# pnnl/ERT-Conditional-Diffusion-Model

Measured on AMD Instinct MI355X. Metric: denoising-steps/sec (64×64, batch 64) at 1/2/4/8 GPUs; conv HBM GB/s vs roofline, higher is better.
Workload: dtype f32

## Files before the change

### ert-conditional-diffusion-model_amd/csrc/unet_conv_wino4s.hip

```cpp
#include <cstdlib>
#include <type_traits>

#include "unet.h"

namespace ertd {
namespace unet {

namespace {

constexpr int NPW = 4;
constexpr int CCH = 8;
constexpr int NX = 36;
constexpr int VKS = 18 * 128;
constexpr int V_FL = 2 * VKS;
constexpr size_t WLDS = (size_t)2 * V_FL * sizeof(float);
constexpr int NRS = 3;
constexpr int GNC_JM = 4;
constexpr int GNC_KM = 6;
constexpr int GNC_TAB = 4096;
#ifndef WINO4S_PPRIO
#define WINO4S_PPRIO 2
#endif
#ifndef WINO4S_PD
#define WINO4S_PD 2
#endif
#ifndef WINO4S_MPRIO
#define WINO4S_MPRIO 1
#endif
#ifndef WINO4S_XCD
#define WINO4S_XCD 1
#endif
#ifndef WINO4S_XCDMAX
#define WINO4S_XCDMAX 2
#endif
#ifndef WINO4S_HALO
#define WINO4S_HALO 1
#endif
#ifndef WINO4S_ABL
#define WINO4S_ABL 0
#endif
using f32x4 = __attribute__((ext_vector_type(4))) float;
using f32x2 = __attribute__((ext_vector_type(2))) float;
using u32x4 = __attribute__((ext_vector_type(4))) unsigned;
using u32x2 = __attribute__((ext_vector_type(2))) unsigned;

__device__ __forceinline__ f32x2 fmac(f32x2 x, float c, f32x2 s) {
  return __builtin_elementwise_fma(x, f32x2{c, c}, s);
}
__device__ __forceinline__ void bt6(const float (&d)[6], float (&o)[6]) {
  const float c = d[4] - d[2], e = d[3] - d[1];
  const float u = d[4] - d[1], v = d[4] + d[1];
  o[0] = __builtin_fmaf(1.5f, e, __builtin_fmaf(-2.f, d[2], d[0] + d[4]));
  o[1] = __builtin_fmaf(2.5f, d[3], __builtin_fmaf(0.5f, d[2], u));
  o[2] = __builtin_fmaf(0.5f, d[3], __builtin_fmaf(-2.5f, d[2], v));
  o[3] = __builtin_fmaf(2.f, e, c);
  o[4] = __builtin_fmaf(-0.5f, e, c);
  o[5] = __builtin_fmaf(1.5f, c, __builtin_fmaf(-2.f, d[3], d[1] + d[5]));
}
__device__ __forceinline__ f32x2 pfma(f32x2 a, float c, f32x2 b) {
  return __builtin_elementwise_fma(a, f32x2{c, c}, b);
}
__device__ __forceinline__ void bt6p(const f32x2 (&d)[6], f32x2 (&o)[6]) {
  const f32x2 c = d[4] - d[2], e = d[3] - d[1];
  const f32x2 u = d[4] - d[1], v = d[4] + d[1];
  o[0] = pfma(e, 1.5f, pfma(d[2], -2.f, d[0] + d[4]));
  o[1] = pfma(d[3], 2.5f, pfma(d[2], 0.5f, u));
  o[2] = pfma(d[3], 0.5f, pfma(d[2], -2.5f, v));
  o[3] = pfma(e, 2.f, c);
  o[4] = pfma(e, -0.5f, c);
  o[5] = pfma(c, 1.5f, pfma(d[3], -2.f, d[1] + d[5]));
}
template <bool DEAD4>
__device__ __forceinline__ void bt6u(const float (&d)[6], float (&o)[6]) {
  const float c = d[4] - d[2], e = d[3] - d[1];
  o[0] = __builtin_fmaf(4.f, d[4], __builtin_fmaf(-5.f, d[2], d[0]));
  o[1] = __builtin_fmaf(-0.25f, d[1] + d[2], d[3] + d[4]);
  o[2] = __builtin_fmaf(0.5f, e, c);
  o[3] = __builtin_fmaf(-0.5f, e, c);
  o[4] = DEAD4 ? 0.f : __builtin_fmaf(0.25f, d[1] - d[2], d[4] - d[3]);
  o[5] = __builtin_fmaf(-1.25f, d[3], __builtin_fmaf(0.25f, d[1], d[5]));
}
template <bool DEAD4>
__device__ __forceinline__ void bt6pu(const f32x2 (&d)[6], f32x2 (&o)[6]) {
  const f32x2 c = d[4] - d[2], e = d[3] - d[1];
  o[0] = pfma(d[4], 4.f, pfma(d[2], -5.f, d[0]));
  o[1] = pfma(d[1] + d[2], -0.25f, d[3] + d[4]);
  o[2] = pfma(e, 0.5f, c);
  o[3] = pfma(e, -0.5f, c);
  o[4] = DEAD4 ? f32x2{0.f, 0.f} : pfma(d[1] - d[2], 0.25f, d[4] - d[3]);
  o[5] = pfma(d[3], -1.25f, pfma(d[1], 0.25f, d[5]));
}
__device__ __forceinline__ void at6u(const f32x2 (&m)[6], f32x2 (&y)[4]) {
  const f32x2 s = m[2] + m[3], d = m[2] - m[3];
  y[0] = (m[0] + m[1]) + s;
  y[1] = fmac(d, 0.5f, m[1]);
  y[2] = fmac(s, 0.25f, m[1]);
  y[3] = fmac(d, 0.125f, m[1] + m[5]);
}
template <int N, bool SHL>
__device__ __forceinline__ f32x2 row_shift0(f32x2 v) {
  constexpr int ctrl = (SHL ? 0x100 : 0x110) + N;
  return f32x2{__int_as_float(__builtin_amdgcn_update_dpp(0, __float_as_int(v.x), ctrl, 0xf, 0xf, true)),
               __int_as_float(__builtin_amdgcn_update_dpp(0, __float_as_int(v.y), ctrl, 0xf, 0xf, true))};
}
template <int N, bool SHL>
__device__ __forceinline__ f32x2 row_shift_keep(f32x2 old, f32x2 v) {
  constexpr int ctrl = (SHL ? 0x100 : 0x110) + N;
  return f32x2{__int_as_float(__builtin_amdgcn_update_dpp(__float_as_int(old.x), __float_as_int(v.x), ctrl, 0xf, 0xf, false)),
               __int_as_float(__builtin_amdgcn_update_dpp(__float_as_int(old.y), __float_as_int(v.y), ctrl, 0xf, 0xf, false))};
}
__device__ __forceinline__ void at6(const f32x2 (&m)[6], f32x2 (&y)[4]) {
  const f32x2 s = m[1] + m[2], d = m[1] - m[2];
  y[0] = (m[0] + s) + (m[3] + m[4]);
  y[1] = fmac(m[3], 0.5f, fmac(m[4], -2.f, d));
  y[2] = fmac(m[3], 0.25f, fmac(m[4], 4.f, s));
  y[3] = fmac(m[3], 0.125f, fmac(m[4], -8.f, d + m[5]));
}

#ifdef WINO4S_STAMP
constexpr int S4_SPW = 64;
__device__ unsigned g_w4s_stamps[256 * 12 * S4_SPW];
#define W4S_STAMP(slot)                                                                            \
  do {                                                                                             \
    if (blockIdx.x < 256 && lane == 0)                                                             \
      g_w4s_stamps[(blockIdx.x * 12 + wave) * S4_SPW + (slot)] = (unsigned)__builtin_amdgcn_s_memtime(); \
  } while (0)
#define W4S_STAMP_ENTRY()                                                                          \
  do {                                                                                             \
    if (blockIdx.x < 256 && lane == 0) {                                                           \
      g_w4s_stamps[(blockIdx.x * 12 + wave) * S4_SPW] = (unsigned)__builtin_amdgcn_s_memrealtime(); \
      g_w4s_stamps[(blockIdx.x * 12 + wave) * S4_SPW + 1] = (unsigned)__builtin_amdgcn_s_memtime(); \
    }                                                                                              \
  } while (0)
#else
#define W4S_STAMP(slot) \
  do {                  \
  } while (0)
#define W4S_STAMP_ENTRY() \
  do {                    \
  } while (0)
#endif

struct Item {
  int cog, blk, half;
};
__device__ __forceinline__ Item item_of(int it, int ncog, int ksp) {
  Item r;
  r.half = it % ksp;
  const int pr = it / ksp;
  r.cog = pr % ncog;
  r.blk = pr / ncog;
  return r;
}

struct ItemWalk {
  int bid, G, ncog, ksp;
  __device__ __forceinline__ Item at(int il) const { return item_of(bid + il * G, ncog, ksp); }
};

constexpr int up25_pair(int xh, int l) { return xh && l >= 3 ? l + 3 : l; }

template <int WO, int ACT, bool UP, int XS, bool GNC>
__global__ __launch_bounds__(64 * (4 * XS + NPW)) void conv_wino4s_kernel(ConvArgs a, int nitems, int ksp) {
  static_assert(!GNC || (XS == 2 && !UP && ACT != ACT_NONE), "GNC: the xi-split GN+act kernel");
  extern __shared__ __attribute__((aligned(16))) float smem[];
  float* vbuf = smem;

  constexpr int TPR = WO / 4;
  constexpr int HW = WO * WO;
  constexpr int TS = TPR * TPR;
  constexpr int WS = UP ? WO / 2 : WO;
  constexpr int HWS = WS * WS;
  constexpr bool UP25 = UP && XS == 2;
  static_assert(TS % 16 == 0 && TPR <= 16, "a 16-tile block is whole tile rows of one sample");
  const int tid = threadIdx.x;
  const int lane = tid & 63;
  const int wave = __builtin_amdgcn_readfirstlane(tid >> 6);
  W4S_STAMP_ENTRY();
  const int Cin = a.Cin, Ca = a.Ca;
  const int nchunk = Cin / CCH / ksp;
  const int ncog = a.Cout / 64;
  const int G = gridDim.x;
  const int bid = (WINO4S_XCD && G % 8 == 0 && ncog <= WINO4S_XCDMAX)
                      ? (int)(blockIdx.x % 8) * (G / 8) + (int)(blockIdx.x / 8) : (int)blockIdx.x;
  const ItemWalk wk{bid, G, ncog, ksp};
  const int nloc = bid < nitems ? (nitems - bid + G - 1) / G : 0;
  float2* const gtab = reinterpret_cast<float2*>(smem + 2 * V_FL + 4 * 2 * 8 * 256);
  const int gtot = nloc * nchunk;

  if (wave >= 4 * XS) {
    __builtin_amdgcn_s_setprio(WINO4S_PPRIO);
    const int q = wave - 4 * XS;
    const int chb = lane >> 5, h = (lane >> 4) & 1, t = lane & 15;
    const int cl = 2 * q + chb;
    const int vwoff = ((((cl >> 2) * 18 + 9 * h) * 4 + (cl & 3)) * 16 + t) * 2;
    const int nbaddr = (lane + 15 - 30 * h) * 4;
    const unsigned choff = (unsigned)(chb * HWS * 4);
    constexpr bool HALO = WINO4S_HALO && !UP && TPR <= 8;
    constexpr int NWR = HALO ? (TPR == 8 ? 5 : 4) : 6;
    float2 raw[NRS][NWR];
    float2 gnv[NRS];
    int gch[NRS];
    f32x4 pad[NRS];
    int cur_g = 0, cur_k = 0, cur_b = 0, cur_il = 0, cur_k0 = 0;
    unsigned roff[NWR];
    f32x4 cur_pad;
    auto set_item = [&](int il) {
      const Item itm = wk.at(il);
      cur_k0 = itm.half * nchunk;
      const int flat0 = itm.blk * 16;
      cur_b = flat0 / TS;
      const int tg = flat0 % TS + t;
      const int ty = tg / TPR, tx = tg - ty * TPR;
      if constexpr (UP) {
#pragma unroll
        for (int r = 0; r < 4; ++r) {
          const int sy = 2 * ty - 1 + r;
          roff[r] = (unsigned)(((sy >= 0 && sy < WS ? sy : 2 * ty) * WS + 2 * tx + h) * 4) + choff;
        }
      } else if constexpr (HALO) {
#pragma unroll
        for (int r = 0; r < 4; ++r) roff[r] = (unsigned)(((4 * ty + r) * WO + 4 * tx + 2 * h) * 4) + choff;
        if constexpr (TPR == 8) {
          const int iy = t < 8 ? 4 * ty - 1 : 4 * ty + 4;
          roff[4] = (unsigned)(((iy >= 0 && iy < WO ? iy : 4 * ty) * WO + 4 * tx + 2 * h) * 4) + choff;
        }
      } else {
#pragma unroll
        for (int r = 0; r < 6; ++r) {
          const int iy = 4 * ty - 1 + r;
          roff[r] = (unsigned)(((iy >= 0 && iy < WO ? iy : 4 * ty) * WO + 4 * tx + 2 * h) * 4) + choff;
        }
      }
      cur_pad = f32x4{ty > 0 ? 1.f : 0.f, ty < TPR - 1 ? 1.f : 0.f,
                      (h ? tx < TPR - 1 : tx > 0) ? 1.f : 0.f, 0.f};
    };
    const int glast = gtot - 1;
    auto load_next = [&](const int set) {
      const int cg = (cur_k0 + cur_k) * CCH + 2 * q;
      pad[set] = cur_pad;
      if constexpr (GNC) gch[set] = cur_il * Cin + cg + chb;
      else if constexpr (ACT != ACT_NONE) gnv[set] = a.gn[(size_t)cur_b * Cin + cg + chb];
      const bool inA = cg < Ca;
      const float* p = inA ? a.srcA + ((size_t)cur_b * Ca + cg) * HWS
                           : a.srcB + ((size_t)cur_b * a.Cb + (cg - Ca)) * HWS;
      const __amdgpu_buffer_rsrc_t rs =
          __builtin_amdgcn_make_buffer_rsrc(const_cast<float*>(p), (short)0, 2 * HWS * 4, 0x00020000);
      if constexpr (UP) {
        float v[4];
#pragma unroll
        for (int r = 0; r < 4; ++r) v[r] = __uint_as_float(__builtin_amdgcn_raw_buffer_load_b32(rs, (int)roff[r], 0, 0));
#pragma unroll
        for (int r = 0; r < 6; ++r) {
          const float u = v[(r + 1) >> 1];
          raw[set][r] = make_float2(u, u);
        }
      } else {
#pragma unroll
        for (int r = 0; r < NWR; ++r) {
          const auto v = __builtin_amdgcn_raw_buffer_load_b64(rs, (int)roff[r], 0, 0);
          raw[set][r] = make_float2(__uint_as_float(v[0]), __uint_as_float(v[1]));
        }
      }
      if (cur_g < glast) {
        ++cur_g;
        if (++cur_k == nchunk) {
          cur_k = 0;
          set_item(++cur_il);
        }
      }
    };
    f32x2 act2[2][6];
    float actn[2][6];
    auto act_stage = [&](const int set, const int ab) {
      if constexpr (GNC) gnv[set] = gtab[gch[set]];
      auto activate = [&](const float2 rw) {
        f32x2 v = f32x2{rw.x, rw.y};
        if constexpr (ACT != ACT_NONE) {
          v = __builtin_elementwise_fma(v, f32x2{gnv[set].x, gnv[set].x}, f32x2{gnv[set].y, gnv[set].y});
          if constexpr (ACT == ACT_GN_SILU) {
            f32x2 e = v * f32x2{-1.44269504088896340736f, -1.44269504088896340736f};
            e = f32x2{__builtin_amdgcn_exp2f(e.x), __builtin_amdgcn_exp2f(e.y)} + f32x2{1.0f, 1.0f};
            v = v * f32x2{__builtin_amdgcn_rcpf(e.x), __builtin_amdgcn_rcpf(e.y)};
          }
        }
        return v;
      };
      f32x2 m[6];
      if constexpr (HALO) {
#pragma unroll
        for (int r = 0; r < 4; ++r) m[1 + r] = activate(raw[set][r]);
        if constexpr (TPR == 8) {
          const f32x2 x = activate(raw[set][4]);
          m[0] = row_shift_keep<TPR, false>(x, m[4]);
          m[5] = row_shift_keep<TPR, true>(x, m[1]);
        } else {
          m[0] = row_shift0<TPR, false>(m[4]);
          m[5] = row_shift0<TPR, true>(m[1]);
        }
      } else {
#pragma unroll
        for (int r = 0; r < 6; ++r) m[r] = activate(raw[set][r]);
      }
      m[0] = m[0] * f32x2{pad[set].x, pad[set].x};
      m[5] = m[5] * f32x2{pad[set].y, pad[set].y};
      if constexpr (UP) bt6pu<UP25>(m, act2[ab]);
      else bt6p(m, act2[ab]);
#pragma unroll
      for (int i = 0; i < 6; ++i) {
        if constexpr (UP25) {
          if (i == 4) {
            actn[ab][i] = 0.f;
            continue;
          }
        }
        const float give = h ? act2[ab][i].y : act2[ab][i].x;
        const float nb = __int_as_float(__builtin_amdgcn_ds_bpermute(nbaddr, __float_as_int(give)));
        actn[ab][i] = nb * pad[set].z;
      }
    };
    auto tr_stage = [&](const int ab, float* vb) {
      float w[6][3];
#pragma unroll
      for (int i = 0; i < 6; ++i) {
        w[i][0] = act2[ab][i].x;
        w[i][1] = act2[ab][i].y;
        w[i][2] = actn[ab][i];
      }
      float row[3][6];
#pragma unroll
      for (int aa = 0; aa < 3; ++aa)
#pragma unroll
        for (int c = 0; c < 3; ++c) {
          const auto sw = __builtin_amdgcn_permlane16_swap(__float_as_uint(w[aa][c]),
                                                           __float_as_uint(w[3 + aa][c]), false, false);
          const int jl = c == 0 ? 1 : (c == 1 ? 2 : 0);
          row[aa][jl] = __uint_as_float(sw[0]);
          row[aa][3 + c] = __uint_as_float(sw[1]);
        }
      float* o = vb + vwoff;
#pragma unroll
      for (int aa = 0; aa < 3; ++aa) {
        float vv[6];
        if constexpr (UP) bt6u<UP25>(row[aa], vv);
        else bt6(row[aa], vv);
        if constexpr (UP25) {
          if (aa == 1 && h) continue;
        }
#pragma unroll
        for (int jp = 0; jp < 6; jp += 2)
          *reinterpret_cast<f32x2*>(o + (aa * 3 + jp / 2) * 128) = f32x2{vv[jp], vv[jp + 1]};
      }
    };
    auto slot = [&](auto sa, auto ab, int g) {
      constexpr int SA = decltype(sa)::value, AB = decltype(ab)::value;
      if constexpr (!(WINO4S_ABL & 1)) {
        tr_stage(AB ^ 1, vbuf + ((g + 1) & 1) * V_FL);
        act_stage(SA, AB);
      }
      load_next(SA);
      if constexpr (!(WINO4S_ABL & 16)) __syncthreads();
    };
    using I0 = std::integral_constant<int, 0>;
    using I1 = std::integral_constant<int, 1>;
    using I2 = std::integral_constant<int, 2>;
    if (gtot > 0) {
      set_item(0);
      load_next(0);
      load_next(1);
      load_next(2);
    }
    if constexpr (GNC) {
      W4S_STAMP(25);
      __syncthreads();
      W4S_STAMP(26);
    }
    if (gtot > 0) {
      act_stage(0, 0);
      tr_stage(0, vbuf);
      load_next(0);
      act_stage(1, 1);
      load_next(1);
    }
    W4S_STAMP(3);
    __syncthreads();
    W4S_STAMP(2);
    int g = 0;
    for (; g + 5 < gtot; g += 6) {
      slot(I2{}, I0{}, g);
      slot(I0{}, I1{}, g + 1);
      slot(I1{}, I0{}, g + 2);
      slot(I2{}, I1{}, g + 3);
      slot(I0{}, I0{}, g + 4);
      slot(I1{}, I1{}, g + 5);
    }
    if (g < gtot) slot(I2{}, I0{}, g);
    if (g + 1 < gtot) slot(I0{}, I1{}, g + 1);
    if (g + 2 < gtot) slot(I1{}, I0{}, g + 2);
    if (g + 3 < gtot) slot(I2{}, I1{}, g + 3);
    if (g + 4 < gtot) slot(I0{}, I0{}, g + 4);
    W4S_STAMP(27);
    return;
  }

  if constexpr (XS == 1) {
  const int cb = wave;
  f32x4 acc[NX];
  const int nks = Cin / 4;
  const __amdgpu_buffer_rsrc_t ru = __builtin_amdgcn_make_buffer_rsrc(
      const_cast<float*>(a.wpk_wino4), (short)0, (int)((size_t)NX * a.Cout * Cin * 4), 0x00020000);
  int u_il = 0, u_ks = 0;
  int u_base = 0;
  auto u_item = [&](int il) {
    const Item itm = wk.at(il);
    u_base = itm.cog * nks * 36864;
  };
  auto u_advance = [&]() {
    if (++u_ks == nks) {
      if (u_il + 1 < nloc) {
        u_ks = 0;
        u_item(++u_il);
      } else {
        u_ks = nks - 1;
      }
    }
  };
  if (nloc > 0) u_item(0);
  f32x2 ub[2][18];
  const int uvoff = lane * 8 + cb * 512;
  auto u_load = [&](f32x2 (&u)[18], const int p) {
    if constexpr ((WINO4S_ABL & 32) != 0) {
      u[p] = u[p] + f32x2{1.f, 1.f};
      return;
    }
    const auto v = __builtin_amdgcn_raw_buffer_load_b64(
        ru, uvoff, (WINO4S_ABL & 2) ? p * 2048 : u_base + u_ks * 36864 + p * 2048, 0);
    u[p] = f32x2{__uint_as_float(v[0]), __uint_as_float(v[1])};
  };
  if (nloc > 0) {
#pragma unroll
    for (int p = 0; p < 18; ++p) u_load(ub[0], p);
    u_advance();
  }
  __syncthreads();
#ifndef WINO4S_XK
#define WINO4S_XK 1
#endif
  auto kstep = [&](const f32x2 (&u)[18], f32x2 (&nx)[18], const float* vs) {
    constexpr int PD = WINO4S_PD;
    f32x2 rb[PD + 1];
#pragma unroll
    for (int p = 0; p < PD; ++p) rb[p] = *reinterpret_cast<const f32x2*>(vs + p * 128);
#pragma unroll
    for (int p = 0; p < 18; ++p) {
      if (p + PD < 18) rb[(p + PD) % (PD + 1)] = *reinterpret_cast<const f32x2*>(vs + (p + PD) * 128);
      const int r = p % (PD + 1);
      if constexpr (WINO4S_ABL & 4) {
        acc[2 * p][0] = __builtin_fmaf(u[p].x, rb[r].x, acc[2 * p][0]);
        acc[2 * p + 1][0] = __builtin_fmaf(u[p].y, rb[r].y, acc[2 * p + 1][0]);
      } else {
        acc[2 * p] = __builtin_amdgcn_mfma_f32_16x16x4f32(u[p].x, rb[r].x, acc[2 * p], 0, 0, 0);
        acc[2 * p + 1] = __builtin_amdgcn_mfma_f32_16x16x4f32(u[p].y, rb[r].y, acc[2 * p + 1], 0, 0, 0);
      }
      u_load(nx, p);
      if (p + PD < 18) __builtin_amdgcn_sched_group_barrier(0x100, 1, 0);
      __builtin_amdgcn_sched_group_barrier(0x008, 2, 0);
      __builtin_amdgcn_sched_group_barrier(0x020, 1, 0);
    }
    u_advance();
  };
  auto chunk2 = [&](const float* vs) {
    constexpr int PD = WINO4S_PD;
    f32x2 rb[PD + 1];
#pragma unroll
    for (int q = 0; q < PD; ++q) rb[q] = *reinterpret_cast<const f32x2*>(vs + q * 128);
#pragma unroll
    for (int q = 0; q < 36; ++q) {
      const int st = q / 18, p = q % 18;
      const int qn = q + PD;
      if (qn < 36) rb[qn % (PD + 1)] = *reinterpret_cast<const f32x2*>(vs + (qn / 18) * VKS + (qn % 18) * 128);
      const int r = q % (PD + 1);
      const f32x2 u = st == 0 ? ub[0][p] : ub[1][p];
      acc[2 * p] = __builtin_amdgcn_mfma_f32_16x16x4f32(u.x, rb[r].x, acc[2 * p], 0, 0, 0);
      acc[2 * p + 1] = __builtin_amdgcn_mfma_f32_16x16x4f32(u.y, rb[r].y, acc[2 * p + 1], 0, 0, 0);
      if (st == 0) u_load(ub[1], p);
      else u_load(ub[0], p);
      if (qn < 36) __builtin_amdgcn_sched_group_barrier(0x100, 1, 0);
      __builtin_amdgcn_sched_group_barrier(0x008, 2, 0);
      __builtin_amdgcn_sched_group_barrier(0x020, 1, 0);
      if (p == 17) u_advance();
    }
  };
  for (int il = 0; il < nloc; ++il) {
#pragma unroll
    for (int x = 0; x < NX; ++x) acc[x] = f32x4{};
    for (int k = 0; k < nchunk; ++k) {
      const int g = il * nchunk + k;
      int ln;
      asm volatile("v_mbcnt_lo_u32_b32 %0, -1, 0\n\tv_mbcnt_hi_u32_b32 %0, -1, %0" : "=v"(ln));
      const float* vb = vbuf + (g & 1) * V_FL + ln * 2;
      if constexpr (WINO4S_XK && !(WINO4S_ABL & 4)) {
        chunk2(vb);
      } else {
        kstep(ub[0], ub[1], vb);
        kstep(ub[1], ub[0], vb + VKS);
      }
#pragma unroll
      for (int x = 0; x < NX; ++x) asm volatile("" : "+v"(acc[x]));
      if constexpr (!(WINO4S_ABL & 16)) __syncthreads();
    }

    if constexpr ((WINO4S_ABL & 8) != 0) {
      if (il == nloc - 1) {
        float sacc = 0.f;
        for (int x = 0; x < NX; ++x) sacc += acc[x][0] + acc[x][3];
        a.out[(size_t)bid * 64 + lane] = sacc;
      }
      continue;
    }
    const Item itm = wk.at(il);
    const int flatw = itm.blk * 16;
    const int smpl = flatw / TS;
    const bool has_eb = a.ebias != nullptr, has_res = a.res != nullptr, has_bias = a.bias != nullptr;
    const unsigned smp = (unsigned)(a.Cout * HW * 4);
    const __amdgpu_buffer_rsrc_t ro = __builtin_amdgcn_make_buffer_rsrc(
        a.out + (size_t)smpl * a.Cout * HW, (short)0, smp, 0x00020000);
    const __amdgpu_buffer_rsrc_t rr = __builtin_amdgcn_make_buffer_rsrc(
        has_res ? const_cast<float*>(a.res) + (size_t)smpl * a.Cout * HW : nullptr, (short)0, smp,
        0x00020000);
    f32x4 y[4][4];
#pragma unroll
    for (int pp = 0; pp < 2; ++pp) {
      f32x2 P[6][4];
#pragma unroll
      for (int i = 0; i < 6; ++i) {
        f32x2 m[6];
#pragma unroll
        for (int j = 0; j < 6; ++j) m[j] = f32x2{acc[6 * i + j][2 * pp], acc[6 * i + j][2 * pp + 1]};
        if constexpr (UP) at6u(m, P[i]);
        else at6(m, P[i]);
      }
#pragma unroll
      for (int x = 0; x < 4; ++x) {
        f32x2 col[6], yc[4];
#pragma unroll
        for (int i = 0; i < 6; ++i) col[i] = P[i][x];
        if constexpr (UP) at6u(col, yc);
        else at6(col, yc);
#pragma unroll
        for (int r = 0; r < 4; ++r) {
          y[2 * pp][r][x] = yc[r].x;
          y[2 * pp + 1][r][x] = yc[r].y;
        }
      }
    }
    int ln;
    asm volatile("v_mbcnt_lo_u32_b32 %0, -1, 0\n\tv_mbcnt_hi_u32_b32 %0, -1, %0" : "=v"(ln));
    const int co0 = itm.cog * 64 + cb * 16 + 4 * (ln >> 4);
    const int tg = flatw % TS + (ln & 15);
    const int ty = tg / TPR, tx = tg - ty * TPR;
    const int vo = (co0 * HW + 4 * ty * WO + 4 * tx) * 4;
#pragma unroll
    for (int i = 0; i < 4; ++i) {
      const float bi = has_bias ? a.bias[co0 + i] : 0.f;
      const float ei = has_eb ? a.ebias[(size_t)smpl * a.eb_stride + co0 + i] : 0.f;
#pragma unroll
      for (int r = 0; r < 4; ++r) {
        y[i][r] = y[i][r] + bi;
        if (has_eb) y[i][r] = y[i][r] + ei;
      }
    }
    __builtin_amdgcn_sched_barrier(0);
    if (has_res) {
      f32x4 rv[4][4];
#pragma unroll
      for (int i = 0; i < 4; ++i)
#pragma unroll
        for (int r = 0; r < 4; ++r)
          rv[i][r] = __builtin_bit_cast(f32x4, __builtin_amdgcn_raw_buffer_load_b128(rr, vo, i * HW * 4 + r * WO * 4, 0));
#pragma unroll
      for (int i = 0; i < 4; ++i)
#pragma unroll
        for (int r = 0; r < 4; ++r) y[i][r] = y[i][r] + rv[i][r];
    }
    if (a.gnp) {
      float2 pr[4];
#pragma unroll
      for (int i = 0; i < 4; ++i) {
        float sm = 0.f;
#pragma unroll
        for (int r = 0; r < 4; ++r) sm += (y[i][r][0] + y[i][r][1]) + (y[i][r][2] + y[i][r][3]);
        sm = row16_sum(sm);
        const float mu = sm * (1.0f / 256.0f);
        float qq = 0.f;
#pragma unroll
        for (int r = 0; r < 4; ++r)
#pragma unroll
          for (int x = 0; x < 4; ++x) {
            const float d = y[i][r][x] - mu;
            qq = __builtin_fmaf(d, d, qq);
          }
        pr[i] = make_float2(sm, row16_sum(qq));
      }
      if ((ln & 15) == 0) {
        const int np = TS / 16, part = (flatw % TS) / 16;
#pragma unroll
        for (int i = 0; i < 4; ++i) {
          float2* d = a.gnp + ((size_t)smpl * a.Cout + co0 + i) * np + part;
          *d = pr[i];
        }
      }
    }
#pragma unroll
    for (int i = 0; i < 4; ++i)
#pragma unroll
      for (int r = 0; r < 4; ++r)
        __builtin_amdgcn_raw_buffer_store_b128(__builtin_bit_cast(u32x4, y[i][r]), ro, vo,
                                               i * HW * 4 + r * WO * 4, 0);
  }
  } else {
  constexpr int NP = 9;
  const int cb = wave & 3, xh = wave >> 2;
#if WINO4S_MPRIO
  if (xh) __builtin_amdgcn_s_setprio(WINO4S_MPRIO);
#endif
  float* xbuf = smem + 2 * V_FL;
  f32x4 acc[2 * NP];
  const int nks = Cin / 4;
  const __amdgpu_buffer_rsrc_t ru = __builtin_amdgcn_make_buffer_rsrc(
      const_cast<float*>(a.wpk_wino4), (short)0, (int)((size_t)NX * a.Cout * Cin * 4), 0x00020000);
  int u_il = 0, u_ks = 0, u_end = 0, u_base = 0;
  auto u_item = [&](int il) {
    const Item itm = wk.at(il);
    u_base = itm.cog * nks * 36864;
    u_ks = itm.half * nchunk * 2;
    u_end = u_ks + nchunk * 2;
  };
  auto u_advance = [&]() {
    if (++u_ks == u_end) {
      if (u_il + 1 < nloc) {
        u_item(++u_il);
      } else {
        u_ks = u_end - 1;
      }
    }
  };
  if (nloc > 0) u_item(0);
  f32x2 ub[2][NP];
  const int uvoff = lane * 8 + cb * 512;
  const int psoff = xh * NP * 2048;
  auto u_load = [&](f32x2 (&u)[NP], const int p) {
    const auto v = __builtin_amdgcn_raw_buffer_load_b64(ru, uvoff, u_base + u_ks * 36864 + psoff + p * 2048, 0);
    u[p] = f32x2{__uint_as_float(v[0]), __uint_as_float(v[1])};
  };
  if (nloc > 0) {
#pragma unroll
    for (int p = 0; p < NP; ++p) {
      if constexpr (UP25) {
        if (xh && p / 3 == 1) continue;
      }
      u_load(ub[0], p);
    }
    u_advance();
  }
  if constexpr (GNC) {
    constexpr int JM = GNC_JM;
    const int ng4 = (a.gnc.groups + 3) / 4;
    int smp[JM], jg[JM], row[JM];
    bool jl[JM];
#pragma unroll
    for (int j = 0; j < JM; ++j) {
      const int job = wave + 4 * XS * j, il = job / ng4;
      jl[j] = il < nloc;
      row[j] = jl[j] ? il : 0;
      jg[j] = job - il * ng4;
      smp[j] = jl[j] ? wk.at(il).blk * 16 / TS : 0;
    }
    gn_group_finalize_regs<JM, GNC_KM>(a.gnc, smp, jg, row, jl, lane, gtab);
    W4S_STAMP(25);
    __syncthreads();
    W4S_STAMP(26);
  }
  __syncthreads();
  W4S_STAMP(2);
  auto chunk2 = [&](const float* vs) {
    constexpr int PD = WINO4S_PD;
    f32x2 rb[PD + 1];
#pragma unroll
    for (int q = 0; q < PD; ++q) rb[q] = *reinterpret_cast<const f32x2*>(vs + (xh * NP + q) * 128);
#pragma unroll
    for (int q = 0; q < 2 * NP; ++q) {
      const int st = q / NP, p = q % NP;
      const int qn = q + PD;
      if (qn < 2 * NP)
        rb[qn % (PD + 1)] = *reinterpret_cast<const f32x2*>(vs + (qn / NP) * VKS + (xh * NP + qn % NP) * 128);
      const int r = q % (PD + 1);
      const f32x2 u = st == 0 ? ub[0][p] : ub[1][p];
      acc[2 * p] = __builtin_amdgcn_mfma_f32_16x16x4f32(u.x, rb[r].x, acc[2 * p], 0, 0, 0);
      acc[2 * p + 1] = __builtin_amdgcn_mfma_f32_16x16x4f32(u.y, rb[r].y, acc[2 * p + 1], 0, 0, 0);
      if (st == 0) u_load(ub[1], p);
      else u_load(ub[0], p);
      if (qn < 2 * NP) __builtin_amdgcn_sched_group_barrier(0x100, 1, 0);
      __builtin_amdgcn_sched_group_barrier(0x008, 2, 0);
      __builtin_amdgcn_sched_group_barrier(0x020, 1, 0);
      if (p == NP - 1) u_advance();
    }
  };
  auto chunk2u = [&](auto xhc, const float* vs) {
    constexpr int XH = decltype(xhc)::value;
    constexpr int NL = XH ? NP - 3 : NP;
    constexpr int PD = WINO4S_PD;
    f32x2 rb[PD + 1];
#pragma unroll
    for (int q = 0; q < PD; ++q) rb[q] = *reinterpret_cast<const f32x2*>(vs + (XH * NP + up25_pair(XH, q)) * 128);
#pragma unroll
    for (int q = 0; q < 2 * NL; ++q) {
      const int st = q / NL, p = up25_pair(XH, q % NL);
      const int qn = q + PD;
      if (qn < 2 * NL)
        rb[qn % (PD + 1)] =
            *reinterpret_cast<const f32x2*>(vs + (qn / NL) * VKS + (XH * NP + up25_pair(XH, qn % NL)) * 128);
      const int r = q % (PD + 1);
      const f32x2 u = st == 0 ? ub[0][p] : ub[1][p];
      const bool both = p % 3 != 2;
      if (both) acc[2 * p] = __builtin_amdgcn_mfma_f32_16x16x4f32(u.x, rb[r].x, acc[2 * p], 0, 0, 0);
      acc[2 * p + 1] = __builtin_amdgcn_mfma_f32_16x16x4f32(u.y, rb[r].y, acc[2 * p + 1], 0, 0, 0);
      if (st == 0) u_load(ub[1], p);
      else u_load(ub[0], p);
      if (qn < 2 * NL) __builtin_amdgcn_sched_group_barrier(0x100, 1, 0);
      if (both) __builtin_amdgcn_sched_group_barrier(0x008, 2, 0);
      else __builtin_amdgcn_sched_group_barrier(0x008, 1, 0);
      __builtin_amdgcn_sched_group_barrier(0x020, 1, 0);
      if (q % NL == NL - 1) u_advance();
    }
  };
  for (int il = 0; il < nloc; ++il) {
#pragma unroll
    for (int x = 0; x < 2 * NP; ++x) acc[x] = f32x4{};
    f32x2 own[4][4];
    auto tail_u = [&](auto xhc) {
      constexpr int XH = decltype(xhc)::value;
#pragma unroll
      for (int pp = 0; pp < 2; ++pp) {
        if (pp) __builtin_amdgcn_sched_barrier(0);
        f32x2 P[3][4], Y[4][4];
#pragma unroll
        for (int i = 0; i < 3; ++i) {
          if (XH && i == 1) continue;
          f32x2 m[6];
#pragma unroll
          for (int j = 0; j < 6; ++j)
            if (j != 4) m[j] = f32x2{acc[6 * i + j][2 * pp], acc[6 * i + j][2 * pp + 1]};
          m[4] = f32x2{0.f, 0.f};
          at6u(m, P[i]);
        }
#pragma unroll
        for (int x = 0; x < 4; ++x) {
          if constexpr (XH == 0) {
            Y[0][x] = P[0][x] + (P[1][x] + P[2][x]);
            Y[1][x] = fmac(P[2][x], 0.5f, P[1][x]);
            Y[2][x] = fmac(P[2][x], 0.25f, P[1][x]);
            Y[3][x] = fmac(P[2][x], 0.125f, P[1][x]);
          } else {
            Y[0][x] = P[0][x];
            Y[1][x] = P[0][x] * f32x2{-0.5f, -0.5f};
            Y[2][x] = P[0][x] * f32x2{0.25f, 0.25f};
            Y[3][x] = fmac(P[0][x], -0.125f, P[2][x]);
          }
        }
        if (pp == XH) {
#pragma unroll
          for (int r = 0; r < 4; ++r)
#pragma unroll
            for (int x = 0; x < 4; ++x) own[r][x] = Y[r][x];
        } else {
          float* xw = xbuf + ((cb * 2 + (XH ^ 1)) * 8) * 256 + lane * 4;
#pragma unroll
          for (int r = 0; r < 4; ++r)
#pragma unroll
            for (int x = 0; x < 4; x += 2)
              *reinterpret_cast<f32x4*>(xw + (r * 2 + x / 2) * 256) =
                  f32x4{Y[r][x].x, Y[r][x].y, Y[r][x + 1].x, Y[r][x + 1].y};
        }
      }
    };
    if (il < 8) W4S_STAMP(3 + 3 * il);
    auto kloop_u = [&](auto xhc) {
      for (int k = 0; k < nchunk; ++k) {
        const int g = il * nchunk + k;
        int ln;
        asm volatile("v_mbcnt_lo_u32_b32 %0, -1, 0\n\tv_mbcnt_hi_u32_b32 %0, -1, %0" : "=v"(ln));
        chunk2u(xhc, vbuf + (g & 1) * V_FL + ln * 2);
#pragma unroll
        for (int x = 0; x < 2 * NP; ++x)
          if (x % 6 != 4) asm volatile("" : "+v"(acc[x]));
        if (k == nchunk - 1) tail_u(xhc);
        __syncthreads();
#ifdef WINO4S_STAMP
        if (g < 32) W4S_STAMP(28 + g);
#endif
      }
    };
    if constexpr (UP25) {
      if (xh == 0) kloop_u(std::integral_constant<int, 0>{});
      else kloop_u(std::integral_constant<int, 1>{});
    } else {
    for (int k = 0; k < nchunk; ++k) {
      const int g = il * nchunk + k;
      int ln;
      asm volatile("v_mbcnt_lo_u32_b32 %0, -1, 0\n\tv_mbcnt_hi_u32_b32 %0, -1, %0" : "=v"(ln));
      chunk2(vbuf + (g & 1) * V_FL + ln * 2);
#pragma unroll
      for (int x = 0; x < 2 * NP; ++x) asm volatile("" : "+v"(acc[x]));
      if (k == nchunk - 1) {
#pragma unroll
        for (int pp = 0; pp < 2; ++pp) {
          f32x2 P[3][4];
#pragma unroll
          for (int i = 0; i < 3; ++i) {
            f32x2 m[6];
#pragma unroll
            for (int j = 0; j < 6; ++j) m[j] = f32x2{acc[6 * i + j][2 * pp], acc[6 * i + j][2 * pp + 1]};
            at6(m, P[i]);
          }
          f32x2 Y[4][4];
#pragma unroll
          for (int x = 0; x < 4; ++x) {
            if (xh == 0) {
              const f32x2 s12 = P[1][x] + P[2][x], d12 = P[1][x] - P[2][x];
              Y[0][x] = P[0][x] + s12;
              Y[1][x] = d12;
              Y[2][x] = s12;
              Y[3][x] = d12;
            } else {
              Y[0][x] = P[0][x] + P[1][x];
              Y[1][x] = fmac(P[0][x], 0.5f, P[1][x] * f32x2{-2.f, -2.f});
              Y[2][x] = fmac(P[0][x], 0.25f, P[1][x] * f32x2{4.f, 4.f});
              Y[3][x] = fmac(P[0][x], 0.125f, fmac(P[1][x], -8.f, P[2][x]));
            }
          }
          if (pp == xh) {
#pragma unroll
            for (int r = 0; r < 4; ++r)
#pragma unroll
              for (int x = 0; x < 4; ++x) own[r][x] = Y[r][x];
          } else {
            float* xw = xbuf + ((cb * 2 + (xh ^ 1)) * 8) * 256 + lane * 4;
#pragma unroll
            for (int r = 0; r < 4; ++r)
#pragma unroll
              for (int x = 0; x < 4; x += 2)
                *reinterpret_cast<f32x4*>(xw + (r * 2 + x / 2) * 256) =
                    f32x4{Y[r][x].x, Y[r][x].y, Y[r][x + 1].x, Y[r][x + 1].y};
          }
        }
      }
      __syncthreads();
#ifdef WINO4S_STAMP
      if (g < 32) W4S_STAMP(28 + g);
#endif
    }
    }
    if (il < 8) W4S_STAMP(4 + 3 * il);
    int ln;
    asm volatile("v_mbcnt_lo_u32_b32 %0, -1, 0\n\tv_mbcnt_hi_u32_b32 %0, -1, %0" : "=v"(ln));
    f32x4 y[2][4];
    {
      const float* xr = xbuf + ((cb * 2 + xh) * 8) * 256 + ln * 4;
#pragma unroll
      for (int r = 0; r < 4; ++r)
#pragma unroll
        for (int x = 0; x < 4; x += 2) {
          const f32x4 o = *reinterpret_cast<const f32x4*>(xr + (r * 2 + x / 2) * 256);
          const f32x2 q0 = own[r][x] + f32x2{o[0], o[1]}, q1 = own[r][x + 1] + f32x2{o[2], o[3]};
          y[0][r][x] = q0.x;
          y[1][r][x] = q0.y;
          y[0][r][x + 1] = q1.x;
          y[1][r][x + 1] = q1.y;
        }
    }
    const Item itm = wk.at(il);
    const int flatw = itm.blk * 16;
    const int smpl = flatw / TS;
    const bool part2 = itm.half != 0;
    const bool has_eb = !part2 && a.ebias != nullptr, has_res = !part2 && a.res != nullptr,
               has_bias = !part2 && a.bias != nullptr;
    const unsigned smp = (unsigned)(a.Cout * HW * 4);
    const __amdgpu_buffer_rsrc_t ro = __builtin_amdgcn_make_buffer_rsrc(
        (part2 ? a.ksplit_buf : a.out) + (size_t)smpl * a.Cout * HW, (short)0, smp, 0x00020000);
    const __amdgpu_buffer_rsrc_t rr = __builtin_amdgcn_make_buffer_rsrc(
        has_res ? const_cast<float*>(a.res) + (size_t)smpl * a.Cout * HW : nullptr, (short)0, smp,
        0x00020000);
    const int co0 = itm.cog * 64 + cb * 16 + 4 * (ln >> 4) + 2 * xh;
    const int tg = flatw % TS + (ln & 15);
    const int ty = tg / TPR, tx = tg - ty * TPR;
    const int vo = (co0 * HW + 4 * ty * WO + 4 * tx) * 4;
#pragma unroll
    for (int i = 0; i < 2; ++i) {
      const float bi = has_bias ? a.bias[co0 + i] : 0.f;
      const float ei = has_eb ? a.ebias[(size_t)smpl * a.eb_stride + co0 + i] : 0.f;
#pragma unroll
      for (int r = 0; r < 4; ++r) {
        y[i][r] = y[i][r] + bi;
        if (has_eb) y[i][r] = y[i][r] + ei;
      }
    }
    __builtin_amdgcn_sched_barrier(0);
    if (has_res) {
      f32x4 rv[2][4];
#pragma unroll
      for (int i = 0; i < 2; ++i)
#pragma unroll
        for (int r = 0; r < 4; ++r)
          rv[i][r] = __builtin_bit_cast(f32x4, __builtin_amdgcn_raw_buffer_load_b128(rr, vo, i * HW * 4 + r * WO * 4, 0));
#pragma unroll
      for (int i = 0; i < 2; ++i)
#pragma unroll
        for (int r = 0; r < 4; ++r) y[i][r] = y[i][r] + rv[i][r];
    }
    if (a.gnp && !part2) {
      float2 pr[2];
#pragma unroll
      for (int i = 0; i < 2; ++i) {
        float sm = 0.f;
#pragma unroll
        for (int r = 0; r < 4; ++r) sm += (y[i][r][0] + y[i][r][1]) + (y[i][r][2] + y[i][r][3]);
        sm = row16_sum(sm);
        const float mu = sm * (1.0f / 256.0f);
        float qq = 0.f;
#pragma unroll
        for (int r = 0; r < 4; ++r)
#pragma unroll
          for (int x = 0; x < 4; ++x) {
            const float d = y[i][r][x] - mu;
            qq = __builtin_fmaf(d, d, qq);
          }
        pr[i] = make_float2(sm, row16_sum(qq));
      }
      if ((ln & 15) == 0) {
        const int np = TS / 16, part = (flatw % TS) / 16;
#pragma unroll
        for (int i = 0; i < 2; ++i) {
          float2* d = a.gnp + ((size_t)smpl * a.Cout + co0 + i) * np + part;
          *d = pr[i];
        }
      }
    }
#pragma unroll
    for (int i = 0; i < 2; ++i)
#pragma unroll
      for (int r = 0; r < 4; ++r)
        __builtin_amdgcn_raw_buffer_store_b128(__builtin_bit_cast(u32x4, y[i][r]), ro, vo,
                                               i * HW * 4 + r * WO * 4, 0);
    if (il < 8) W4S_STAMP(5 + 3 * il);
  }
  W4S_STAMP(27);
  }

}

}

#ifdef WINO4S_STAMP
extern "C" int ertd_diag_wino4s_stamps(unsigned* host, size_t n) {
  const size_t cap = sizeof(g_w4s_stamps) / sizeof(unsigned);
  return (int)hipMemcpyFromSymbol(host, HIP_SYMBOL(g_w4s_stamps), (n < cap ? n : cap) * sizeof(unsigned), 0,
                                  hipMemcpyDeviceToHost);
}
extern "C" int ertd_diag_wino4s_stamps_clear() {
  static unsigned zero[256 * 12 * S4_SPW];
  return (int)hipMemcpyToSymbol(HIP_SYMBOL(g_w4s_stamps), zero, sizeof(zero), 0, hipMemcpyHostToDevice);
}
#endif

namespace {

template <int WO, int ACT, bool UP, int XS>
hipError_t launch_wo4x(const ConvArgs& a, hipStream_t s, const WinoRoute& r) {
  constexpr size_t lds = WLDS + (XS == 2 ? (size_t)4 * 2 * 8 * 256 * sizeof(float) : 0);
  const int nitems = r.items, grid = r.grid, ksp = r.ksplit;
  if (ksp != 1 && (a.gnc.pa || XS != 2)) return hipErrorInvalidValue;
  if constexpr (XS == 2 && !UP && ACT != ACT_NONE) {
    if (a.gnc.pa) {
      const int nlocmax = (nitems + grid - 1) / grid;
      const size_t ldsg = lds + (size_t)nlocmax * a.Cin * sizeof(float2);
      static std::atomic<unsigned long long> attr{0};
      set_max_lds_once((const void*)conv_wino4s_kernel<WO, ACT, UP, XS, true>,
                       (int)(lds + GNC_TAB * sizeof(float2)), attr);
      conv_wino4s_kernel<WO, ACT, UP, XS, true><<<grid, 64 * (4 * XS + NPW), ldsg, s>>>(a, nitems, ksp);
      return hipGetLastError();
    }
  }
  if (a.gnc.pa) return hipErrorInvalidValue;
  {
    static std::atomic<unsigned long long> attr{0};
    set_max_lds_once((const void*)conv_wino4s_kernel<WO, ACT, UP, XS, false>, (int)lds, attr);
    conv_wino4s_kernel<WO, ACT, UP, XS, false><<<grid, 64 * (4 * XS + NPW), lds, s>>>(a, nitems, ksp);
  }
  hipError_t e = hipGetLastError();
  if (e != hipSuccess || ksp == 1) return e;
  return launch_add_inplace(a.out, a.ksplit_buf, r.kbuf_floats, s);
}

template <int WO, int ACT, bool UP>
hipError_t launch_wo4s(const ConvArgs& a, hipStream_t s, const WinoRoute& r) {
  if (wino4s_xs() == 2 && a.Cin >= 16) return launch_wo4x<WO, ACT, UP, 2>(a, s, r);
  return launch_wo4x<WO, ACT, UP, 1>(a, s, r);
}

template <int ACT, bool UP>
hipError_t launch_act4s(const ConvArgs& a, hipStream_t s, const WinoRoute& r) {
  switch (a.Wo) {
    case 16: return launch_wo4s<16, ACT, UP>(a, s, r);
    case 32: return launch_wo4s<32, ACT, UP>(a, s, r);
    case 64: return launch_wo4s<64, ACT, UP>(a, s, r);
    default: return hipErrorInvalidValue;
  }
}

}

bool wino_gnc_ok(const WinoRoute& r, int Cin, int Wo, const GnPartArgs& g) {
  static const int env = [] {
    return ERTD_KNOB("UNET_GNC", 3);
  }();
  if (r.kernel != WinoRoute::F4S || r.ksplit != 1) return false;
  if (!env || wino4s_xs() != 2 || Cin < 16) return false;
  if (!g.pa || g.groups < 1 || g.Ca + g.Cb != Cin || Cin % g.groups || g.npa < 1 ||
      (g.Cb > 0 && (!g.pb || g.npb < 1)) || g.HW != Wo * Wo || g.HW % g.npa ||
      (g.Cb > 0 && g.HW % g.npb))
    return false;
  const int nloc = (r.items + r.grid - 1) / r.grid;
  const int cpg = Cin / g.groups;
  const int np = g.npa > g.npb ? g.npa : g.npb;
  if (env == 2 && nloc > 1) return false;
  if (env == 3 && nloc > 2) return false;
  return nloc > 0 && nloc * ((g.groups + 3) / 4) <= 8 * GNC_JM && cpg <= GN_LPG &&
         cpg * np <= GN_LPG * GNC_KM && nloc * Cin <= GNC_TAB;
}

hipError_t launch_conv_wino4s(int act, const ConvArgs& a, hipStream_t s, const WinoRoute& r) {
  if (r.kernel == WinoRoute::F4S_UP)
    return act == ACT_NONE ? launch_act4s<ACT_NONE, true>(a, s, r) : hipErrorInvalidValue;
  if (r.kernel != WinoRoute::F4S) return hipErrorInvalidValue;
  switch (act) {
    case ACT_NONE: return launch_act4s<ACT_NONE, false>(a, s, r);
    case ACT_GN_SILU: return launch_act4s<ACT_GN_SILU, false>(a, s, r);
    case ACT_GN: return launch_act4s<ACT_GN, false>(a, s, r);
    default: return hipErrorInvalidValue;
  }
}

}
}
```

Baseline: 266.7.

## Prefetch residual, bias and ebias into exchange LDS during producer mainloop

In the xi-split non-upsample Winograd conv kernel, producer waves now load the residual tile plus bias/ebias during the channel-chunk loop. They spread the loads across chunk slots and write res+bias+ebias into the LDS exchange buffer ahead of the epilogue. The MFMA waves then accumulate their cross-half partials onto that buffer and skip the per-element residual and bias loads in the epilogue. This moves residual HBM reads off the critical epilogue path, at the cost of extra producer work, registers and LDS traffic, and it relies on the exchange buffer not being overwritten.

```diff
diff --git a/ert-conditional-diffusion-model_amd/csrc/unet_conv_wino4s.hip b/ert-conditional-diffusion-model_amd/csrc/unet_conv_wino4s.hip
--- a/ert-conditional-diffusion-model_amd/csrc/unet_conv_wino4s.hip
+++ b/ert-conditional-diffusion-model_amd/csrc/unet_conv_wino4s.hip
@@ -35,6 +35,9 @@
 #endif
 #ifndef WINO4S_HALO
 #define WINO4S_HALO 1
+#endif
+#ifndef WINO4S_RESX
+#define WINO4S_RESX 1
 #endif
 #ifndef WINO4S_ABL
 #define WINO4S_ABL 0
@@ -172,6 +175,7 @@
   constexpr int WS = UP ? WO / 2 : WO;
   constexpr int HWS = WS * WS;
   constexpr bool UP25 = UP && XS == 2;
+  constexpr bool RESX = WINO4S_RESX && XS == 2 && !UP;
   static_assert(TS % 16 == 0 && TPR <= 16, "a 16-tile block is whole tile rows of one sample");
   const int tid = threadIdx.x;
   const int lane = tid & 63;
@@ -352,6 +356,69 @@
           *reinterpret_cast<f32x2*>(o + (aa * 3 + jp / 2) * 128) = f32x2{vv[jp], vv[jp + 1]};
       }
     };
+    f32x4 rres[4];
+    float rbi[2], rei[2];
+    int pch = -1;
+    struct RCur {
+      int il, k, cog, flat0;
+      bool q;
+    };
+    RCur sc{0, 0, 0, 0, false};
+    const bool res_fit = RESX && a.res != nullptr && nchunk >= 3;
+    const bool res_lag = nchunk >= 6;
+    auto rc_item = [&](RCur& c, int il) {
+      c.il = il;
+      c.k = 0;
+      c.q = false;
+      if (res_fit && il < nloc) {
+        const Item itm = wk.at(il);
+        c.q = itm.half == 0;
+        c.cog = itm.cog;
+        c.flat0 = itm.blk * 16;
+      }
+    };
+    auto rc_next = [&](RCur& c) {
+      if (++c.k == nchunk) rc_item(c, c.il + 1);
+    };
+    auto res_slot = [&](int ch) { return 1 + ((ch * (nchunk - 2)) >> 2); };
+    auto res_ch = [&](int k) {
+      int ch = -1;
+#pragma unroll
+      for (int c = 0; c < 4; ++c) ch = res_slot(c) == k ? c : ch;
+      return ch;
+    };
+    auto res_issue = [&](const RCur& c, int ch) {
+      const int smpl = c.flat0 / TS;
+      const int tg = c.flat0 % TS + t;
+      const int ty = tg / TPR, tx = tg - ty * TPR;
+      const int col = 4 * (lane >> 4);
+      const int co = c.cog * 64 + q * 16 + (ch & 2);
+      const int r0 = 2 * (ch & 1);
+      const __amdgpu_buffer_rsrc_t rs = __builtin_amdgcn_make_buffer_rsrc(
+          const_cast<float*>(a.res) + (size_t)smpl * a.Cout * HW, (short)0, a.Cout * HW * 4, 0x00020000);
+      const int vo = (col * HW + 4 * ty * WO + 4 * tx) * 4;
+#pragma unroll
+      for (int i = 0; i < 2; ++i) {
+#pragma unroll
+        for (int rr = 0; rr < 2; ++rr)
+          rres[i * 2 + rr] = __builtin_bit_cast(
+              f32x4, __builtin_amdgcn_raw_buffer_load_b128(rs, vo, ((co + i) * HW + (r0 + rr) * WO) * 4, 0));
+        rbi[i] = a.bias ? a.bias[co + col + i] : 0.f;
+        rei[i] = a.ebias ? a.ebias[(size_t)smpl * a.eb_stride + co + col + i] : 0.f;
+      }
+    };
+    auto res_write = [&](int ch) {
+      float* xw = smem + 2 * V_FL + ((q * 2 + (ch >> 1)) * 8 + (ch & 1) * 4) * 256 + lane * 4;
+      const float be0 = rbi[0] + rei[0], be1 = rbi[1] + rei[1];
+#pragma unroll
+      for (int rr = 0; rr < 2; ++rr)
+#pragma unroll
+        for (int x = 0; x < 4; x += 2) {
+          const f32x4 c0 = rres[rr], c1 = rres[2 + rr];
+          *reinterpret_cast<f32x4*>(xw + (rr * 2 + x / 2) * 256) =
+              f32x4{c0[x] + be0, c1[x] + be1, c0[x + 1] + be0, c1[x + 1] + be1};
+        }
+    };
     auto slot = [&](auto sa, auto ab, int g) {
       constexpr int SA = decltype(sa)::value, AB = decltype(ab)::value;
       if constexpr (!(WINO4S_ABL & 1)) {
@@ -359,6 +426,20 @@
         act_stage(SA, AB);
       }
       load_next(SA);
+      if constexpr (RESX) {
+        if (pch >= 0) res_write(pch);
+        if (!res_lag && sc.q) {
+#pragma nounroll
+          for (int ch = 0; ch < 4; ++ch)
+            if (res_slot(ch) == sc.k) {
+              res_issue(sc, ch);
+              res_write(ch);
+            }
+        }
+        rc_next(sc);
+        pch = res_lag && sc.q ? res_ch(sc.k) : -1;
+        if (pch >= 0) res_issue(sc, pch);
+      }
       if constexpr (!(WINO4S_ABL & 16)) __syncthreads();
     };
     using I0 = std::integral_constant<int, 0>;
@@ -381,6 +462,9 @@
       load_next(0);
       act_stage(1, 1);
       load_next(1);
+      if constexpr (RESX) {
+        rc_item(sc, 0);
+      }
     }
     W4S_STAMP(3);
     __syncthreads();
@@ -738,6 +822,8 @@
 #pragma unroll
     for (int x = 0; x < 2 * NP; ++x) acc[x] = f32x4{};
     f32x2 own[4][4];
+    bool resx = false;
+    if constexpr (RESX) resx = a.res != nullptr && nchunk >= 3 && wk.at(il).half == 0;
     auto tail_u = [&](auto xhc) {
       constexpr int XH = decltype(xhc)::value;
 #pragma unroll
@@ -844,6 +930,15 @@
             for (int r = 0; r < 4; ++r)
 #pragma unroll
               for (int x = 0; x < 4; ++x) own[r][x] = Y[r][x];
+          } else if (resx) {
+            float* xw = xbuf + ((cb * 2 + (xh ^ 1)) * 8) * 256 + lane * 4;
+#pragma unroll
+            for (int r = 0; r < 4; ++r)
+#pragma unroll
+              for (int x = 0; x < 4; x += 2) {
+                f32x4* p = reinterpret_cast<f32x4*>(xw + (r * 2 + x / 2) * 256);
+                *p = *p + f32x4{Y[r][x].x, Y[r][x].y, Y[r][x + 1].x, Y[r][x + 1].y};
+              }
           } else {
             float* xw = xbuf + ((cb * 2 + (xh ^ 1)) * 8) * 256 + lane * 4;
 #pragma unroll
@@ -883,8 +978,8 @@
     const int flatw = itm.blk * 16;
     const int smpl = flatw / TS;
     const bool part2 = itm.half != 0;
-    const bool has_eb = !part2 && a.ebias != nullptr, has_res = !part2 && a.res != nullptr,
-               has_bias = !part2 && a.bias != nullptr;
+    const bool has_eb = !part2 && !resx && a.ebias != nullptr, has_res = !part2 && !resx && a.res != nullptr,
+               has_bias = !part2 && !resx && a.bias != nullptr;
     const unsigned smp = (unsigned)(a.Cout * HW * 4);
     const __amdgpu_buffer_rsrc_t ro = __builtin_amdgcn_make_buffer_rsrc(
         (part2 ? a.ksplit_buf : a.out) + (size_t)smpl * a.Cout * HW, (short)0, smp, 0x00020000);
```

New measurement: 259.7. 2.6% lower.
